# shiivashaakeri/Dynamic-Programming-MultiAgent-Trajectory-Optimiziation

Hardware: AMD Instinct MI355X
Metric: SCvx-iterations/sec, N agents x K=50 nodes (N=1024 per GPU) (higher is better)
Workload: dtype f64

## Files before the change

dynamic-programming-multiagent-trajectory-optimiziation_amd/csrc/qp_factor_phase.hpp:

```cpp
#pragma once
#include "qp_access.hpp"
#include "wave_ops.hpp"

namespace scvx {


struct QPRep {
    int L, R, B, O, G;
    double b1, b2, acc;
};
__device__ __forceinline__ QPRep qp_decode(const int (&d)[4], int one, int lsink, int jnk) {
    QPRep q;
    q.L = d[0] & 0x7FFF;
    q.R = d[1] & 0x7FFF;
    const int bk = d[3] >> 16;
    q.B = bk ? (d[3] & 0x7FFF) : one;
    q.b1 = bk == 1 ? 1.0 : 0.0;
    q.b2 = bk == 2 ? 1.0 : 0.0;
    const int O = d[2];
    const bool on = O >= 0, acc = on && ((O >> 15) & 1);
    q.O = (on && !acc) ? (O & 0x7FFF) : lsink;
    q.acc = acc ? 1.0 : 0.0;
    const int g = on ? (O >> 17) - 1 : -1;
    q.G = (g >= 0 ? g : jnk) * 8;
    return q;
}

template <int KK>
__device__ __forceinline__ double qp_dot(const double* lds, int L, int R) {
    const double* lp = lds + L;
    const double* rp = lds + R;
    double acc0 = 0.0, acc1 = 0.0;
#pragma unroll
    for (int k = 0; k < KK; ++k) {
        if (k & 1) acc1 = fma(lp[k], rp[k], acc1); else acc0 = fma(lp[k], rp[k], acc0);
    }
    return acc0 + acc1;
}

template <int KK, int NREP, int ALO = 0, int AHI = WAVE * NREP>
__device__ __forceinline__ void qp_phase(double* lds, const QPRep (&d)[NREP], double blast, const QPBuf& wb, int fbo,
                                         double (&areg)[NREP]) {
    double val[NREP];
#pragma unroll
    for (int r = 0; r < NREP; ++r)
        val[r] = fma(lds[d[r].B], d[r].b1 + blast * d[r].b2, qp_dot<KK>(lds, d[r].L, d[r].R));
#pragma unroll
    for (int r = 0; r < NREP; ++r) {
        lds[d[r].O] = val[r];
        if (WAVE * r < AHI && WAVE * r + WAVE > ALO) areg[r] = fma(d[r].acc, val[r], areg[r]);
        wb.st(d[r].G, fbo, val[r]);
    }
}

struct QPRepC {
    int LR, BO, GF;
    __device__ __forceinline__ int L() const { return LR & 0xFFFF; }
    __device__ __forceinline__ int R() const { return LR >> 16; }
    __device__ __forceinline__ int B() const { return BO & 0xFFFF; }
    __device__ __forceinline__ int O() const { return BO >> 16; }
    __device__ __forceinline__ int G() const { return GF & 0xFFFF; }
    __device__ __forceinline__ int F() const { return GF >> 16; }
};
__device__ __forceinline__ QPRepC qp_decode_c(const int (&d)[4], int one, int lsink, int jnk) {
    QPRepC q;
    const int L = d[0] & 0x7FFF, R = d[1] & 0x7FFF;
    const int bk = d[3] >> 16;
    const int B = bk ? (d[3] & 0x7FFF) : one;
    const int O = d[2];
    const bool on = O >= 0, acc = on && ((O >> 15) & 1);
    const int Oo = on ? (O & 0x7FFF) : lsink;
    const int g = on ? (O >> 17) - 1 : -1;
    const int G = (g >= 0 ? g : jnk) * 8;
    const int F = bk | (acc ? 4 : 0);
    q.LR = L | (R << 16);
    q.BO = B | (Oo << 16);
    q.GF = G | (F << 16);
    return q;
}
template <int KK, int NREP, int ALO, int AHI>
__device__ __forceinline__ void qp_phase_c(double* lds, const QPRepC* d, double blast, const QPBuf& wb,
                                           int fbo, double (&areg)[NREP]) {
    const QPRepC* q = d;
    double val[NREP];
#pragma unroll
    for (int r = 0; r < NREP; ++r) {
        const int bk = q[r].F() & 3;
        const double bm = (bk == 1 ? 1.0 : 0.0) + blast * (bk == 2 ? 1.0 : 0.0);
        val[r] = fma(lds[q[r].B()], bm, qp_dot<KK>(lds, q[r].L(), q[r].R()));
    }
#pragma unroll
    for (int r = 0; r < NREP; ++r) {
        lds[q[r].O()] = val[r];
        if (WAVE * r < AHI && WAVE * r + WAVE > ALO) areg[r] = fma((q[r].F() & 4) ? 1.0 : 0.0, val[r], areg[r]);
        wb.st(q[r].G(), fbo, val[r]);
    }
}

}
```

dynamic-programming-multiagent-trajectory-optimiziation_amd/csrc/qp_ipm.hpp:

```cpp
#pragma once
#ifndef __HIPCC_RTC__
#include <hip/hip_runtime.h>

#include "common.hpp"
#endif
#include <type_traits>

#include "qp_consts.hpp"
#include "qp_factor_phase.hpp"

namespace scvx {

template <int NX_, int NU_, int NB_, int NO_, int NC_, int VC_ = 0>
struct QPCfg {
    static constexpr QPLay L = qp_layout(NX_, NU_, NB_, NO_, NC_, VC_);
    static_assert(qp_class_error(NX_, NU_, NB_, NO_, NC_, VC_, 2, QP_LDS_DEVICE) == nullptr, "class outside the kernel's limits");
};

struct QPFlagsRT {
    static constexpr bool spec = false;
    static constexpr int has_final = 0, fix_last_input = 0, ineq_last = 0, has_soc = 0, has_coll = 0, n_obs = 0, n_box = 0;
    static constexpr int box_idx(int) { return 0; }
};
template <int FIN, int FIXU, int INEQL, int SOC, int COLL, int NOBS, int NBOX, int B0 = 0, int B1 = 0>
// ... 204 lines not shown
            }
#pragma unroll
            for (int e = 0; e < NX * NU; ++e) pst(C::L.gC + e, Cp[e]);
        }
        const int pd = T.pos_dim;
        double xb[3] = {0, 0, 0};
        for (int i = 0; i < pd; ++i) xb[i] = act ? a.Xref[(agent * K + t) * NX + i] : 0.0;
#pragma unroll
        for (int o = 0; o < NO; ++o) {
            double d[3] = {0, 0, 0}, nr = 0.0, bo = 0.0;
            if (o < nobs) {
                bo = T.obs_radius[o];
#pragma unroll
                for (int i = 0; i < 3; ++i) {
                    d[i] = i < pd ? xb[i] - T.obs_center[o][i] : 0.0;
                    nr += d[i] * d[i];
                }
                nr = sqrt(nr) + 1e-6;
#pragma unroll
                for (int i = 0; i < 3; ++i) {
                    d[i] = d[i] / nr;
                    bo += i < pd ? d[i] * T.obs_center[o][i] : 0.0;
                }
            }
#pragma unroll
            for (int i = 0; i < 3; ++i) cst(C::L.C_SOFT + o * 4 + i, d[i]);
            cst(C::L.C_SOFT + o * 4 + 3, bo);
        }
#pragma unroll
        for (int c = 0; c < NC; ++c) {
            double g[4] = {0, 0, 0, 0};
            if (c < ccount) {
                const double* src = a.coll_rows + ((agent * K + t) * T.j_max + c) * (pd + 1);
                for (int i = 0; i < pd; ++i) g[i] = src[i];
                g[3] = src[pd];
            }
#pragma unroll
            for (int i = 0; i < 4; ++i) cst(C::L.C_SOFT + (NO + c) * 4 + i, g[i]);
        }
#pragma unroll
        for (int j = 0; j < NU; ++j) cst(C::L.C_UB + j, act ? a.Uref[(agent * K + t) * NU + j] : 0.0);
        if (warm) {
            if (lane < 2 * NX) lds[V_YI + lane] = wld(vt, C::L.C_WY * colb);
        } else {
#pragma unroll
            for (int i = 0; i < NX; ++i) {
                cst(C::L.C_Z + i, act ? a.Xref[(agent * K + t) * NX + i] : 0.0);
                cst(C::L.C_Y + i, 0.0);
            }
#pragma unroll
            for (int j = 0; j < NU; ++j) cst(C::L.C_Z + NX + j, act ? a.Uref[(agent * K + t) * NU + j] : 0.0);
#pragma unroll
            for (int g = 0; g < NG; ++g) cst(C::L.C_AV + g, 0.0);
#pragma unroll
            for (int i = 0; i < NV; ++i) { cst(C::L.C_VN + i, 0.0); cst(C::L.C_VE + i, 0.0); }
            if (lane < NX) { lds[V_YI + lane] = 0.0; lds[V_YF + lane] = 0.0; }
        }
        if (lane == 0) lds[V_ONE] = 1.0;
        if (lane < 16) lds[V_ST + lane] = 0.0;
    }
    auto issue_cp = [&](double* Cp) __attribute__((always_inline)) {
#pragma unroll
        for (int e = 0; e < NX * NU; ++e) Cp[e] = wld(vcur - 8, (C::L.C_DT + NX * NX + NX * NU + e) * colb);
    };
    auto take_cp = [&](double* Cp) __attribute__((always_inline)) {
        hold(Cp, NX * NU);
#pragma unroll
        for (int e = 0; e < NX * NU; ++e) Cp[e] = (t > 0) ? Cp[e] : 0.0;
    };
    auto load_cp = [&](double* Cp) __attribute__((always_inline)) {
        issue_cp(Cp);
        take_cp(Cp);
    };
#ifndef QP_RT_STEPS
#define QP_RT_STEPS 15
#endif
    constexpr bool RT_ON = NX <= 8 && NS <= 8 && NV == 0;
    constexpr bool RT_A = RT_ON && (QP_RT_STEPS & 1), RT_B = RT_ON && (QP_RT_STEPS & 2),
                   RT_C = RT_ON && (QP_RT_STEPS & 4), RT_F = RT_ON && (QP_RT_STEPS & 8);

    constexpr int PFN = (PKT + WAVE - 1) / WAVE;
    auto factor = [&](auto phi_issue) __attribute__((always_inline)) -> bool {
        constexpr int E1 = 2 * NX * NX + 2 * NX * NU + 2 * NX, E2 = NX * NX + NU * NX + NU * NU, E4 = 4 * NX * NX;
        constexpr int R1 = (E1 + WAVE - 1) / WAVE, R2 = (E2 + WAVE - 1) / WAVE, R4 = (E4 + WAVE - 1) / WAVE;
        int d1[R1][4], d2[R2][4], d4[R4][4];
        {
            const int sink = C::L.F_SINK;
            const int ln = qp_opaque(lane);
#pragma unroll
            for (int rep = 0; rep < R1; ++rep) {
                int o = ln + rep * WAVE, L = 0, R = 0, O = -1, B = 0;
                if (o < NX * NX) {
                    const int i = o / NX, j = o % NX;
                    L = C::L.F_PP + i * NX; R = C::L.P_A + j * NX; O = C::L.F_T1 + j * NX + i;
                } else if ((o -= NX * NX) < NX * NU) {
                    const int i = o / NU, j = o % NU;
                    L = C::L.F_PP + i * NX; R = C::L.P_BT + j * NX; O = C::L.F_T2 + j * NX + i;
                } else if ((o -= NX * NU) < NX * NX) {
                    const int i = o / NX, j = o % NX;
                    L = C::L.P_A + i * NX; R = C::L.F_PIP + j * NX; O = C::L.F_W1 + o;
                    B = (i == j) ? (V_ONE | (2 << 16)) : 0;
                } else if ((o -= NX * NX) < NU * NX) {
                    const int i = o / NX, j = o % NX;
                    L = C::L.P_BT + i * NX; R = C::L.F_PIP + j * NX;
                    O = (C::L.F_W2 + j * NU + i) | ((C::L.B_W2 + o + 1) << 17);
                    B = (C::L.P_C + i * NX + j) | (1 << 15) | (2 << 16);
                } else if ((o -= NU * NX) < NX) {
                    L = C::L.F_PP + o * NX; R = C::L.P_E; O = sink | ((C::L.B_U + o + 1) << 17);
                } else if ((o -= NX) < NX) {
                    L = C::L.F_PIP + o * NX; R = C::L.P_E; O = (V_XE + o) | (1 << 15);
                }
                d1[rep][0] = L; d1[rep][1] = R; d1[rep][2] = O; d1[rep][3] = B;
            }
#pragma unroll
            for (int rep = 0; rep < R2; ++rep) {
                int o = ln + rep * WAVE, L = 0, R = 0, O = -1, B = 0;
                if (o < NX * NX) {
                    const int i = o / NX, j = o % NX, p = i < j ? i : j, q = i < j ? j : i;
                    L = C::L.P_A + p * NX; R = C::L.F_T1 + q * NX; O = C::L.F_QH + o;
                    B = (C::L.P_Q + p * NX + q) | (1 << 15) | (1 << 16);
                } else if ((o -= NX * NX) < NU * NX) {
                    const int i = o / NX, j = o % NX;
                    L = C::L.P_BT + i * NX; R = C::L.F_T1 + j * NX; O = C::L.F_SH + j * NU + i;
                    B = (C::L.P_S + j * NU + i) | (1 << 15) | (1 << 16);
                } else if ((o -= NU * NX) < NU * NU) {
                    const int i = o / NU, j = o % NU, p = i < j ? i : j, q = i < j ? j : i;
                    L = C::L.P_BT + p * NX; R = C::L.F_T2 + q * NX; O = C::L.F_RH + o;
                    B = (C::L.P_R + p * NU + q) | (1 << 15) | (1 << 16);
                }
                d2[rep][0] = L; d2[rep][1] = R; d2[rep][2] = O; d2[rep][3] = B;
            }
#pragma unroll
            for (int rep = 0; rep < R4; ++rep) {
                int o = ln + rep * WAVE, L = 0, R = 0, O = -1, B = 0;
                if (o < NX * NX) {
                    const int i = o / NX, j = o % NX, p = i < j ? i : j, q = i < j ? j : i;
                    L = C::L.F_SH + p * NU; R = C::L.F_KK + q * NU;
                    O = (C::L.F_PP + o) | ((C::L.B_P + o + 1) << 17); B = (C::L.F_QH + p * NX + q) | (1 << 16);
                } else if ((o -= NX * NX) < NX * NX) {
                    const int i = o / NX, j = o % NX;
                    L = C::L.F_SH + i * NU; R = C::L.F_KK + (NX + j) * NU;
                    O = (C::L.F_PIP + j * NX + i) | ((C::L.B_PI + o + 1) << 17); B = (C::L.F_W1 + o) | (1 << 16);
                } else if ((o -= NX * NX) < NX * NX) {
                    const int i = o / NX, j = o % NX, p = i < j ? i : j, q = i < j ? j : i;
                    L = C::L.F_W2 + p * NU; R = C::L.F_KK + (NX + q) * NU; O = (V_M + o) | (1 << 15);
                } else if ((o -= NX * NX) < NX * NX) {
                    const int i = o / NX, j = o % NX;
                    L = C::L.P_BTR + i * NU; R = C::L.F_KK + j * NU;
                    O = (C::L.NV > 0 ? C::L.F_ACLC + j * NX + i : sink) | ((C::L.B_ACL + o + 1) << 17);
                    B = (C::L.P_A + j * NX + i) | (1 << 15) | (1 << 16);
                }
                d4[rep][0] = L; d4[rep][1] = R; d4[rep][2] = O; d4[rep][3] = B;
            }
        }
        constexpr bool CMP = NX > 8;
        constexpr int RT = R1 + R2 + R4;
        static_assert(!CMP || RT == C::L.NREP, "descriptor table size (QPLay::dtab_doubles, the host's workspace size)");
        const int DTB = FBB + K * C::L.FBS * 8;
        QPRep q1[CMP ? 1 : R1], q2[CMP ? 1 : R2], q4[CMP ? 1 : R4];
        double a1[R1], a2[R2], a4[R4];
        constexpr int R0 = (NX * NX + WAVE - 1) / WAVE;
        double amv[R0];
#pragma unroll
        for (int r = 0; r < R0; ++r) amv[r] = 0.0;
        auto tab_st = [&](int r, const QPRepC& q) __attribute__((always_inline)) {
            qp_u4 w;
            w.x = (unsigned)q.LR; w.y = (unsigned)q.BO; w.z = (unsigned)q.GF; w.w = 0u;
            wb.st4(qp_opaque(lane) * 16, DTB + r * WAVE * 16, w);
        };
        auto tab_ld = [&](int r, int vo) __attribute__((always_inline)) -> QPRepC {
            const qp_u4 w = wb.ld4(vo, DTB + r * WAVE * 16);
            QPRepC q;
            q.LR = (int)w.x; q.BO = (int)w.y; q.GF = (int)w.z;
            return q;
        };
#pragma unroll
        for (int r = 0; r < R1; ++r) {
            if constexpr (CMP) tab_st(r, qp_decode_c(d1[r], V_ONE, C::L.F_SINK, C::L.B_JNK));
            else q1[r] = qp_decode(d1[r], V_ONE, C::L.F_SINK, C::L.B_JNK);
            a1[r] = 0.0;
        }
#pragma unroll
        for (int r = 0; r < R2; ++r) {
            if constexpr (CMP) tab_st(R1 + r, qp_decode_c(d2[r], V_ONE, C::L.F_SINK, C::L.B_JNK));
            else q2[r] = qp_decode(d2[r], V_ONE, C::L.F_SINK, C::L.B_JNK);
            a2[r] = 0.0;
        }
#pragma unroll
        for (int r = 0; r < R4; ++r) {
            if constexpr (CMP) tab_st(R1 + R2 + r, qp_decode_c(d4[r], V_ONE, C::L.F_SINK, C::L.B_JNK));
            else q4[r] = qp_decode(d4[r], V_ONE, C::L.F_SINK, C::L.B_JNK);
            a4[r] = 0.0;
        }
        for (int e = lane; e < NX * NX; e += WAVE) { lds[C::L.F_PP + e] = 0.0; lds[C::L.F_PIP + e] = 0.0; lds[V_M + e] = 0.0; }
        if (lane < NX) lds[V_XE + lane] = 0.0;
        if (lane == 0) { lds[V_FLAG] = 0.0; lds[V_SANY] = 0.0; }
        __syncthreads();
        constexpr int FPD = NX > 8 ? 2 : 3;
        double pf[FPD][PFN];
        int pfo[C::L.DPK ? 1 : PFN];
        if constexpr (!C::L.DPK) {
#pragma unroll
            for (int k = 0; k < PFN; ++k) {
                const int e = qp_opaque(lane) + WAVE * k;
                const int g = e < PKT ? qp_gsrc<C::L>(e) : -1;
                pfo[k] = g >= 0 ? g * 8 : QP_OOB;
            }
        }
        auto pf_load = [&](int ts, double* b) __attribute__((always_inline)) {
            if constexpr (C::L.DPK) {
                const int vo = qp_opaque(lane) * 8;
#pragma unroll
                for (int k = 0; k < PFN; ++k) b[k] = wb.ld(vo, PKB + (ts > 0 ? ts : 0) * C::L.GPK * 8 + k * WAVE * 8);
            } else {
#pragma unroll
                for (int k = 0; k < PFN; ++k) b[k] = wb.ld(pfo[k], PKB + (ts > 0 ? ts : 0) * C::L.GPK * 8);
            }
        };
        auto pf_store = [&](int ts, const double* b) __attribute__((always_inline)) {
            const int sl = NX > 8 ? qp_opaque(lane) : lane;
#pragma unroll
            for (int k = 0; k < PFN; ++k) {
                const int e = sl + WAVE * k;
                lds[e < PKT ? C::L.F_RING + e : C::L.F_SINK] = b[k];
            }
        };
        if constexpr (FPD == 3) {
            pf_load(K - 1, pf[0]);
            pf_load(K - 2, pf[1]);
            pf_load(K - 3, pf[2]);
            pf_store(K - 1, pf[0]);
            pf_load(K - 4, pf[0]);
        } else {
            pf_load(K - 1, pf[0]);
            pf_load(K - 2, pf[1]);
            pf_store(K - 1, pf[0]);
            pf_load(K - 3, pf[0]);
        }
        wsync();
        bool bad = false;
        auto stage = [&](auto lastc, int ts, double* nb, const double* cb) __attribute__((always_inline)) {
            constexpr bool last = decltype(lastc)::value;
            const double blast = last ? 1.0 : 0.0;
            const int fbo = FBB + ts * C::L.FBS * 8;
            const int sl = NX > 8 ? qp_opaque(lane) : lane;
            QPRepC qs[CMP ? RT : 1];
            if constexpr (CMP) {
                const int vo = qp_opaque(lane) * 16;
#pragma unroll
                for (int r = 0; r < RT; ++r) qs[r] = tab_ld(r, vo);
            }
            pf_load(ts - FPD, nb);
            double dfmr = 0.0;
            if constexpr (C::L.STF) dfmr = lds[C::L.F_RING + C::L.P_FD + C::L.NTR + 1 + C::L.NFO];
            if constexpr (C::L.NV > 0) {
                const int c = sl < 4 * NX ? sl : 0, blk = c / NX, cc = c - blk * NX;
                const int base = (blk == 1 ? C::L.F_PIP : C::L.F_PP) + cc * NX;
                const double keep = blk == 2 ? 0.0 : 1.0;
                const double dcc = lds[C::L.F_RING + C::L.P_D + cc];
                const double diag = (blk == 2 ? 1.0 : 0.0) + (blk == 0 ? dcc : 0.0);
                double col[NX];
#pragma unroll
                for (int i = 0; i < NX; ++i) col[i] = fma(keep, lds[base + i], qp_mask(i, cc) * diag);
#pragma unroll
                for (int k = 0; k < NX; ++k) {
                    double pv[NX];
#pragma unroll
                    for (int i = 0; i < NX; ++i) pv[i] = readlane_d(col[i], k);
                    bad |= !(pv[k] > 0.0);
                    const double rk = col[k] / pv[k];
#pragma unroll
                    for (int i = 0; i < NX; ++i) col[i] = (i == k) ? rk : fma(-pv[i], rk, col[i]);
                }
                const bool own = sl >= NX && sl < 4 * NX;
                const int gcol = blk == 1 ? C::L.B_YPI : (blk == 2 ? C::L.B_GI : C::L.B_YP);
#pragma unroll
                for (int i = 0; i < NX; ++i) {
                    const int lo = !own ? C::L.F_SINK + i
                                        : (blk == 1 ? C::L.F_YPI + cc * NX + i
                                                    : (blk == 2 ? C::L.F_Z + i * NX + cc : C::L.F_YP + cc * NX + i));
                    lds[lo] = blk == 2 ? col[i] * dcc : col[i];
                    wb.st((own ? gcol + cc * NX + i : C::L.B_JNK) * 8, fbo, col[i]);
                }
                wsync();
#pragma unroll
                for (int r = 0; r < R0; ++r) {
                    const int o = sl + r * WAVE, oo = o < NX * NX ? o : 0, i = oo / NX, j = oo - i * NX;
                    const double pt = 0.5 * (lds[C::L.F_RING + C::L.P_D + i] * lds[C::L.F_YP + j * NX + i] +
                                             lds[C::L.F_RING + C::L.P_D + j] * lds[C::L.F_YP + i * NX + j]);
                    const double mv = qp_dot<NX>(lds, C::L.F_PIP + i * NX, C::L.F_YPI + j * NX);
                    amv[r] -= o < NX * NX ? mv : 0.0;
                    lds[o < NX * NX ? C::L.F_PP + o : C::L.F_SINK] = pt;
                }
                wsync();
#pragma unroll
                for (int r = 0; r < R0; ++r) {
                    const int o = sl + r * WAVE, oo = o < NX * NX ? o : 0;
                    const double v = lds[C::L.F_RING + C::L.P_D + (oo % NX)] * lds[C::L.F_YPI + oo];
                    lds[o < NX * NX ? C::L.F_PIP + o : C::L.F_SINK] = v;
                }
                wsync();
            }
            pstamp(15);
            if constexpr (CMP) qp_phase_c<NX, R1, E1 - NX, E1>(lds, qs, blast, wb, fbo, a1);
            else qp_phase<NX, R1, E1 - NX, E1>(lds, q1, blast, wb, fbo, a1);
            wsync();
            pstamp(11);
            if constexpr (CMP) qp_phase_c<NX, R2, 0, 0>(lds, qs + R1, blast, wb, fbo, a2);
            else qp_phase<NX, R2, 0, 0>(lds, q2, blast, wb, fbo, a2);
            wsync();
            pstamp(12);
            {
                const bool fx = last && fix_last;
                auto ph3 = [&](auto candc) __attribute__((always_inline)) {
                constexpr bool CAND = decltype(candc)::value;
                constexpr int PM = C::L.PM, PMA = C::L.PMA;
                double Lm[NU * NU], dinv[NU];
#pragma unroll
                for (int e = 0; e < NU * NU; ++e) Lm[e] = lds[C::L.F_RH + e];
                int sfi[PMA];
                double sfd[PMA];
#pragma unroll
                for (int i = 0; i < PMA; ++i) { sfi[i] = -1; sfd[i] = 1.0; }
                bool stg = false;
                if constexpr (C::L.STF && CAND) {
                    constexpr int NTR = C::L.NTR, FS = C::L.F_RING + C::L.P_FD + NTR;
                    {
                    double dnf = 0.0;
#pragma unroll
                    for (int j = 0; j < NU; ++j) dnf = fmax(dnf, fabs(Lm[j * NU + j]));
                    const double thr = QP_STIFF * dnf;
                    {
                        int e = 0;
#pragma unroll
                        for (int i = 0; i < NU; ++i) {
                            Lm[i * NU + i] += lds[FS];
#pragma unroll
                            for (int j = i + 1; j < NU; ++j, ++e) {
                                const double o = lds[FS + 1 + e];
                                Lm[i * NU + j] += o;
                                Lm[j * NU + i] += o;
                            }
                        }
                    }
                    if (__builtin_amdgcn_readfirstlane((int)(dfmr > thr && !fx))) {
                        double Df[NTR];
                        int cnt = 0;
#pragma unroll
                        for (int f = 0; f < NTR; ++f) {
                            Df[f] = lds[C::L.F_RING + C::L.P_FD + f];
                            const bool above = Df[f] > thr;
#pragma unroll
                            for (int i = 0; i < PM; ++i) {
                                sfi[i] = (above && cnt == i) ? f : sfi[i];
                                sfd[i] = (above && cnt == i) ? Df[f] : sfd[i];
                            }
                            cnt += above ? 1 : 0;
                        }
                        bool opp = false;
#pragma unroll
                        for (int i = 0; i < PM; ++i)
#pragma unroll
                            for (int k = i + 1; k < PM; ++k) opp |= sfi[i] >= 0 && sfi[k] >= 0 && (sfi[i] ^ sfi[k]) == NTR - 1;
                        const bool use = cnt <= PM && !opp;
#pragma unroll
                        for (int i = 0; i < PM; ++i) {
                            sfi[i] = use ? sfi[i] : -1;
                            sfd[i] = use ? sfd[i] : 1.0;
                        }
                        if (use) {
#pragma unroll
                            for (int e = 0; e < NU * NU; ++e) Lm[e] = lds[C::L.F_RH + e];
#pragma unroll
                            for (int f = 0; f < NTR; ++f) {
                                bool st = false;
#pragma unroll
                                for (int i = 0; i < PM; ++i) st |= sfi[i] == f;
                                const double d = st ? 0.0 : Df[f];
#pragma unroll
                                for (int i = 0; i < NU; ++i)
#pragma unroll
                                    for (int j = 0; j < NU; ++j) Lm[i * NU + j] += (((f >> i) ^ (f >> j)) & 1) ? -d : d;
                            }
                        }
                        stg = __builtin_amdgcn_readfirstlane((int)use) != 0;
                        if (stg && sl == 0) lds[V_SANY] = 1.0;
                    }
                    }
                }
#ifdef QP_STF_DEBUG
                double Lm0[NU * NU];
#pragma unroll
                for (int e = 0; e < NU * NU; ++e) Lm0[e] = Lm[e];
#endif
                double dmax = 0.0;
#pragma unroll
                for (int j = 0; j < NU; ++j) dmax = fmax(dmax, fabs(Lm[j * NU + j]));
                const double dmin = 1e-13 * dmax + 1e-300;
                bool nan = dmax != dmax;
#pragma unroll
                for (int j = 0; j < NU; ++j) {
                    double d = Lm[j * NU + j];
#pragma unroll
                    for (int k = 0; k < j; ++k) d -= Lm[j * NU + k] * Lm[j * NU + k] * Lm[k * NU + k];
                    nan |= d != d;
                    d = d > dmin ? d : dmin;
                    Lm[j * NU + j] = d;
                    double rq = __builtin_amdgcn_rcp(d);
                    rq = fma(fma(-d, rq, 1.0), rq, rq);
                    dinv[j] = fma(fma(-d, rq, 1.0), rq, rq);
#pragma unroll
                    for (int i = j + 1; i < NU; ++i) {
                        double v = Lm[i * NU + j];
#pragma unroll
                        for (int k = 0; k < j; ++k) v -= Lm[i * NU + k] * Lm[j * NU + k] * Lm[k * NU + k];
                        Lm[i * NU + j] = v * dinv[j];
                    }
                }
                bad |= nan;
                if (fx) {
#pragma unroll
                    for (int e = 0; e < NU * NU; ++e) Lm[e] = (e / NU == e % NU) ? 1.0 : 0.0;
#pragma unroll
                    for (int j = 0; j < NU; ++j) dinv[j] = 1.0;
                }
                auto ldl_solve = [&](double* x) __attribute__((always_inline)) {
#pragma unroll
                    for (int i = 0; i < NU; ++i) {
#pragma unroll
                        for (int k = 0; k < i; ++k) x[i] -= Lm[i * NU + k] * x[k];
                    }
#pragma unroll
                    for (int i = 0; i < NU; ++i) x[i] *= dinv[i];
#pragma unroll
                    for (int i = NU - 1; i >= 0; --i) {
#pragma unroll
                        for (int k = i + 1; k < NU; ++k) x[i] -= Lm[k * NU + i] * x[k];
                    }
                };
                double Wm[NU * PMA], Ci[PMA * PMA];
#pragma unroll
                for (int e = 0; e < NU * PMA; ++e) Wm[e] = 0.0;
#pragma unroll
                for (int e = 0; e < PMA * PMA; ++e) Ci[e] = (e / PMA == e % PMA) ? 1.0 : 0.0;
                if (C::L.STF && CAND && stg) {
#pragma unroll
                    for (int i = 0; i < PM; ++i) {
                        double w[NU];
#pragma unroll
                        for (int j = 0; j < NU; ++j) w[j] = sfi[i] < 0 ? 0.0 : (((sfi[i] >> j) & 1) ? -1.0 : 1.0);
                        ldl_solve(w);
#pragma unroll
                        for (int j = 0; j < NU; ++j) Wm[j * PM + i] = w[j];
                    }
                    double Cm[PMA * PMA];
#pragma unroll
                    for (int i = 0; i < PM; ++i)
#pragma unroll
                        for (int k = 0; k < PM; ++k) {
                            double v = (i == k) ? (sfi[i] < 0 ? 1.0 : 1.0 / sfd[i]) : 0.0;
#pragma unroll
                            for (int j = 0; j < NU; ++j)
                                v += (sfi[i] < 0 ? 0.0 : (((sfi[i] >> j) & 1) ? -1.0 : 1.0)) * Wm[j * PM + k];
                            Cm[i * PM + k] = v;
                        }
#ifdef QP_STF_DEBUG
                    double Cm0[PMA * PMA];
#pragma unroll
                    for (int e = 0; e < PM * PM; ++e) Cm0[e] = Cm[e];
#endif
#pragma unroll
                    for (int e = 0; e < PM * PM; ++e) Ci[e] = (e / PM == e % PM) ? 1.0 : 0.0;
#pragma unroll
                    for (int k = 0; k < PM; ++k) {
                        const double pv = Cm[k * PM + k];
                        bad |= !(pv > 0.0 && __builtin_isfinite(pv));
#ifdef QP_STF_DEBUG
                        if (sl == 0 && !(pv > 0.0 && __builtin_isfinite(pv))) {
                            printf("STF agent %lld stage %d pivot %d = %.6e | C %.6e %.6e %.6e %.6e | sfi %d %d sfd %.3e %.3e | "
                                   "W %.3e %.3e %.3e %.3e %.3e %.3e\n", agent, ts, k, pv, Cm0[0], Cm0[1], Cm0[2], Cm0[3],
                                   sfi[0], sfi[PMA > 1 ? 1 : 0], sfd[0], sfd[PMA > 1 ? 1 : 0], Wm[0], Wm[1], Wm[2],
                                   Wm[3 % (NU * PMA)], Wm[4 % (NU * PMA)], Wm[5 % (NU * PMA)]);
                            printf("STF agent %lld stage %d R0 (folded, before LDL) %.6e %.6e %.6e | %.6e %.6e %.6e | %.6e %.6e %.6e"
                                   " | Rhat %.6e %.6e %.6e %.6e %.6e %.6e %.6e %.6e %.6e | dinv %.6e %.6e %.6e | L %.6e %.6e %.6e\n",
                                   agent, ts, Lm0[0], Lm0[1 % (NU * NU)], Lm0[2 % (NU * NU)], Lm0[3 % (NU * NU)],
                                   Lm0[4 % (NU * NU)], Lm0[5 % (NU * NU)], Lm0[6 % (NU * NU)], Lm0[7 % (NU * NU)],
                                   Lm0[8 % (NU * NU)], lds[C::L.F_RH + 0], lds[C::L.F_RH + 1], lds[C::L.F_RH + 2],
                                   lds[C::L.F_RH + 3], lds[C::L.F_RH + 4 % (NU * NU)], lds[C::L.F_RH + 5 % (NU * NU)],
                                   lds[C::L.F_RH + 6 % (NU * NU)], lds[C::L.F_RH + 7 % (NU * NU)], lds[C::L.F_RH + 8 % (NU * NU)], dinv[0],
                                   dinv[1 % NU], dinv[2 % NU], Lm[3 % (NU * NU)], Lm[6 % (NU * NU)], Lm[7 % (NU * NU)]);
                            double Df8[8];
                            for (int f = 0; f < 8; ++f) Df8[f] = f < C::L.NTR ? lds[C::L.F_RING + C::L.P_FD + f] : 0.0;
                            printf("STF agent %lld stage %d facets D %.3e %.3e %.3e %.3e %.3e %.3e %.3e %.3e\n", agent, ts,
                                   Df8[0], Df8[1], Df8[2], Df8[3], Df8[4], Df8[5], Df8[6], Df8[7]);
                        }
#endif
                        const double rp = 1.0 / pv;
#pragma unroll
                        for (int j = 0; j < PM; ++j) { Cm[k * PM + j] *= rp; Ci[k * PM + j] *= rp; }
#pragma unroll
                        for (int i = 0; i < PM; ++i) {
                            if (i == k) continue;
                            const double f = Cm[i * PM + k];
#pragma unroll
                            for (int j = 0; j < PM; ++j) {
                                Cm[i * PM + j] = fma(-f, Cm[k * PM + j], Cm[i * PM + j]);
                                Ci[i * PM + j] = fma(-f, Ci[k * PM + j], Ci[i * PM + j]);
                            }
                        }
                    }
#pragma unroll
                    for (int e = 0; e < PM * PM; ++e) bad |= !__builtin_isfinite(Ci[e]);
#ifdef QP_STF_DEBUG
                    for (int e = 0; e < PM * PM; ++e)
                        if (sl == 0 && !__builtin_isfinite(Ci[e])) printf("STF agent %lld stage %d Ci[%d] = %.6e\n", agent, ts, e, Ci[e]);
#endif
                }
                {
                    const bool kl = sl < 2 * NX;
                    const int c = kl ? sl : 0;
                    const int off = c < NX ? C::L.F_SH + c * NU : C::L.F_W2 + (c - NX) * NU;
                    double x[NU];
#pragma unroll
                    for (int i = 0; i < NU; ++i) x[i] = lds[off + i];
                    ldl_solve(x);
                    if constexpr (C::L.STF) {
                        double gx[PMA], zc[PMA];
#pragma unroll
                        for (int i = 0; i < PMA; ++i) zc[i] = 0.0;
                        if (CAND && stg) {
#pragma unroll
                        for (int i = 0; i < PM; ++i) {
                            double v = 0.0;
#pragma unroll
                            for (int j = 0; j < NU; ++j)
                                v += (sfi[i] < 0 ? 0.0 : (((sfi[i] >> j) & 1) ? -1.0 : 1.0)) * x[j];
                            gx[i] = v;
                        }
#pragma unroll
                        for (int i = 0; i < PM; ++i) {
                            double v = 0.0;
#pragma unroll
                            for (int k = 0; k < PM; ++k) v = fma(Ci[i * PM + k], gx[k], v);
                            zc[i] = v;
                        }
#pragma unroll
                        for (int j = 0; j < NU; ++j)
#pragma unroll
                            for (int i = 0; i < PM; ++i) x[j] = fma(-Wm[j * PM + i], zc[i], x[j]);
                        }
                        const int gb = c < NX ? C::L.B_GAM + c : C::L.B_GAK + c - NX;
#pragma unroll
                        for (int i = 0; i < PM; ++i) wb.st((kl ? gb + i * NX : C::L.B_JNK) * 8, fbo, fx ? 0.0 : -zc[i]);
                    }
                    const int g = c < NX ? C::L.B_K + c : C::L.B_KAP + c - NX;
#pragma unroll
                    for (int i = 0; i < NU; ++i) {
                        const double v = fx ? 0.0 : -x[i];
                        lds[kl ? C::L.F_KK + c * NU + i : C::L.F_SINK] = v;
                        wb.st((kl ? g + i * NX : C::L.B_JNK) * 8, fbo, v);
                    }
                }
                {
                    double v = 0.0;
#pragma unroll
                    for (int e = 0; e < NU * NU; ++e) {
                        const int ei = e / NU, ej = e % NU;
                        if (ei >= ej) v = (sl == e) ? (ei > ej ? Lm[e] : dinv[ei]) : v;
                    }
                    wb.st((sl < NU * NU ? C::L.B_LD + sl : C::L.B_JNK) * 8, fbo, v);
                }
                if constexpr (C::L.STF) {
                    double v = 0.0;
#pragma unroll
                    for (int e = 0; e < NU * PM; ++e) v = (sl == e) ? Wm[e] : v;
#pragma unroll
                    for (int e = 0; e < PM * PM; ++e) v = (sl == NU * PM + e) ? Ci[e] : v;
#pragma unroll
                    for (int e = 0; e < PM; ++e) v = (sl == NU * PM + PM * PM + e) ? (double)sfi[e] : v;
                    wb.st((sl < C::L.NSMB ? C::L.B_WS + sl : C::L.B_JNK) * 8, fbo, v);
                }
                };
                if constexpr (C::L.STF) {
                    if (__builtin_amdgcn_readfirstlane((int)(dfmr > 0.0))) ph3(std::true_type{});
                    else ph3(std::false_type{});
                } else {
                    ph3(std::false_type{});
                }
            }
            wsync();
            pstamp(13);
            if constexpr (CMP) qp_phase_c<NU, R4, 2 * NX * NX, 3 * NX * NX>(lds, qs + R1 + R2, blast, wb, fbo, a4);
            else qp_phase<NU, R4, 2 * NX * NX, 3 * NX * NX>(lds, q4, blast, wb, fbo, a4);
            if (ts > 0) pf_store(ts - 1, cb);
            wsync();
            pstamp(14);
            if constexpr (C::L.NV > 0) {
#pragma unroll
                for (int r = 0; r < R0; ++r) {
                    const int o = sl + r * WAVE, oo = o < NX * NX ? o : 0, i = oo / NX, j = oo - i * NX;
                    const double v = qp_dot<NX>(lds, C::L.F_Z + i * NX, C::L.F_ACLC + j * NX);
                    wb.st((o < NX * NX ? C::L.B_ACL2 + o : C::L.B_JNK) * 8, fbo, v);
                }
                wsync();
            }
        };
        int ts = K - 1;
        if constexpr (FPD == 3) {
            stage(std::true_type{}, ts, pf[0], pf[1]);
            --ts;
            while (ts >= 0) {
                stage(std::false_type{}, ts, pf[1], pf[2]);
                if (--ts < 0) break;
                stage(std::false_type{}, ts, pf[2], pf[0]);
                if (--ts < 0) break;
                stage(std::false_type{}, ts, pf[0], pf[1]);
                --ts;
            }
        } else {
            stage(std::true_type{}, ts, pf[0], pf[1]);
            --ts;
            while (ts >= 0) {
                stage(std::false_type{}, ts, pf[1], pf[0]);
                if (--ts < 0) break;
                stage(std::false_type{}, ts, pf[0], pf[1]);
                --ts;
            }
        }
        if (bad) lds[V_FLAG] = 1.0;
        if constexpr (CMP) {
            const int vo = qp_opaque(lane) * 16;
#pragma unroll
            for (int r = 0; r < R1; ++r) {
                if (WAVE * r < E1 && WAVE * r + WAVE > E1 - NX) {
                    const QPRepC q = tab_ld(r, vo);
                    if (q.F() & 4) lds[q.O()] = a1[r];
                }
            }
#pragma unroll
            for (int r = 0; r < R4; ++r) {
                if (WAVE * r < 3 * NX * NX && WAVE * r + WAVE > 2 * NX * NX) {
                    const QPRepC q = tab_ld(R1 + R2 + r, vo);
                    if (q.F() & 4) lds[q.O()] = a4[r];
                }
            }
        } else {
#pragma unroll
            for (int r = 0; r < R1; ++r)
                if (d1[r][2] >= 0 && ((d1[r][2] >> 15) & 1)) lds[d1[r][2] & 0x7FFF] = a1[r];
#pragma unroll
            for (int r = 0; r < R4; ++r)
                if (d4[r][2] >= 0 && ((d4[r][2] >> 15) & 1)) lds[d4[r][2] & 0x7FFF] = a4[r];
        }
        wsync();
        if constexpr (C::L.NV > 0) {
#pragma unroll
            for (int r = 0; r < R0; ++r) {
                const int o = lane + r * WAVE;
                if (o < NX * NX) lds[V_M + o] += amv[r];
            }
            wsync();
        }
        for (int e = lane; e < NX * NX; e += WAVE) lds[V_PI0 + e] = lds[C::L.F_PIP + (e % NX) * NX + e / NX];
        if constexpr (NX > 8) {
            if (fin) {
                const int j = lane < NX ? lane : 0;
                double col[NX];
#pragma unroll
                for (int i = 0; i < NX; ++i) col[i] = lds[V_M + i * NX + j];
#pragma unroll
                for (int k = 0; k < NX; ++k) {
                    double ck[NX];
#pragma unroll
                    for (int i = 0; i < NX; ++i) ck[i] = readlane_d(col[i], k);
                    int p = k;
                    double best = fabs(ck[k]);
#pragma unroll
                    for (int i = k + 1; i < NX; ++i) {
                        const double v = fabs(ck[i]);
                        if (v > best) { best = v; p = i; }
                    }
                    if (lane == 0) lds[V_PIV + k] = (double)p;
#pragma unroll
                    for (int i = k + 1; i < NX; ++i) {
                        const double m = qp_mask(i, p);
                        const double dlt = m * (col[i] - col[k]);
                        col[k] += dlt;
                        col[i] -= dlt;
                    }
#pragma unroll
                    for (int i = 0; i < NX; ++i) ck[i] = readlane_d(col[i], k);
                    const double d = ck[k];
                    if (lane == 0 && (d == 0.0 || d != d)) lds[V_FLAG] = 2.0;
                    const double inv = d != 0.0 ? 1.0 / d : 0.0;
#pragma unroll
                    for (int i = k + 1; i < NX; ++i) {
                        const double f = ck[i] * inv;
                        col[i] = (j == k) ? f : ((j > k) ? col[i] - f * col[k] : col[i]);
                    }
                }
                if (lane < NX)
#pragma unroll
                    for (int i = 0; i < NX; ++i) lds[V_M + i * NX + j] = col[i];
            }
        } else {
        if (fin && lane == 0) {
            double Mr[NX * NX];
#pragma unroll
            for (int e = 0; e < NX * NX; ++e) Mr[e] = lds[V_M + e];
#pragma unroll
            for (int k = 0; k < NX; ++k) {
                int p = k;
                double best = fabs(Mr[k * NX + k]);
#pragma unroll
                for (int i = k + 1; i < NX; ++i) {
                    const double v = fabs(Mr[i * NX + k]);
                    if (v > best) { best = v; p = i; }
                }
                lds[V_PIV + k] = (double)p;
#pragma unroll
                for (int i = k + 1; i < NX; ++i) {
                    const double m = qp_mask(i, p);
#pragma unroll
                    for (int j = 0; j < NX; ++j) {
                        const double dlt = m * (Mr[i * NX + j] - Mr[k * NX + j]);
                        Mr[k * NX + j] += dlt;
                        Mr[i * NX + j] -= dlt;
                    }
                }
                const double d = Mr[k * NX + k];
                if (d == 0.0 || d != d) lds[V_FLAG] = 2.0;
                const double inv = d != 0.0 ? 1.0 / d : 0.0;
#pragma unroll
                for (int i = k + 1; i < NX; ++i) {
                    const double f = Mr[i * NX + k] * inv;
                    Mr[i * NX + k] = f;
#pragma unroll
                    for (int j = k + 1; j < NX; ++j) Mr[i * NX + j] -= f * Mr[k * NX + j];
                }
            }
#pragma unroll
            for (int e = 0; e < NX * NX; ++e) lds[V_M + e] = Mr[e];
        }
        }
        wsync();
        if constexpr (C::L.CHK) {
            const ChunkC cc = chunk_coords();
            const int ch = cc.ch, ce = cc.ce, cs0 = cc.cs0, cs1 = cc.cs1;
            const bool cact = cc.act;
            double ar[QP_CLM][NX], ph[NX];
#pragma unroll
            for (int j = 0; j < QP_CLM; ++j) {
                const int tj = cs0 + j;
                const int vo = (cact && j < CL && tj < cs1) ? (C::L.B_CH + ce * NX) * 8 + tj * C::L.FBS * 8 : QP_OOB;
#pragma unroll
                for (int k = 0; k < NX; ++k) {
                    if constexpr (NX % 2 == 0) { if (!(k & 1)) wld2(&ar[j][k], vo, FBB, k * 8); }
                    else ar[j][k] = wld(vo, FBB, k * 8);
                }
            }
            phi_issue();
#pragma unroll
            for (int c = 0; c < NX; ++c) ph[c] = (c == ce) ? 1.0 : 0.0;
#pragma unroll
            for (int j = 0; j < QP_CLM; ++j) {
                if (j < CL) {
                    double nw[NX];
#pragma unroll
                    for (int c = 0; c < NX; ++c) nw[c] = 0.0;
#pragma unroll
                    for (int k = 0; k < NX; ++k)
#pragma unroll
                        for (int c = 0; c < NX; ++c) nw[c] = fma(ar[j][k], oct_bcast_d(ph[c], k), nw[c]);
                    const bool ok = cs0 + j < cs1;
#pragma unroll
                    for (int c = 0; c < NX; ++c) ph[c] = ok ? nw[c] : ph[c];
                }
            }
#pragma unroll
            for (int c = 0; c < NX; ++c) lds[cact ? V_PHI + ch * NX * NX + ce * NX + c : C::L.F_SINK] = ph[c];
            wsync();
        }
        return lds[V_FLAG] == 0.0;
    };

    auto solve = [&](const double* q, const double* r, const double* dv, double* dzo, double* dyo, double* dno,
                     const double* rhs_s, double* fnu) __attribute__((always_inline)) {
        constexpr int PM = C::L.PM, PMA = C::L.PMA;
        double g0[PMA];
#pragma unroll
        for (int i = 0; i < PMA; ++i) { g0[i] = 0.0; fnu[i] = 0.0; }
        fresh();
        if (act) {
            double g[NX], u[NX];
            ldb(u, C::L.B_U, NX);
            if constexpr (NV > 0) {
                double Y[NX * NX];
                ldb(Y, C::L.B_YP, NX * NX);
                hold(u, NX);
                hold(Y, NX * NX);
#pragma unroll
                for (int j = 0; j < NX; ++j)
#pragma unroll
                    for (int i = 0; i < NX; ++i) u[j] = fma(-Y[j * NX + i], dv[i], u[j]);
            }
            double Kt[NU * NX], Ac[NX * NX];
            ldb(Kt, C::L.B_K, NU * NX);
            ldb(Ac, C::L.B_ACL, NX * NX);
            hold(Kt, NU * NX);
            hold(u, NX);
            hold(Ac, NX * NX);
#pragma unroll
            for (int i = 0; i < NX; ++i) g[i] = q[i];
            if constexpr (C::L.STF) {
                if (stf_any()) {
                    double Gm[PMA * NX];
                    ldb(Gm, C::L.B_GAM, PM * NX);
                    hold(Gm, PM * NX);
#pragma unroll
                    for (int i = 0; i < PM; ++i)
#pragma unroll
                        for (int j = 0; j < NX; ++j) g[j] = fma(-Gm[i * NX + j], rhs_s[i], g[j]);
                }
            }
#pragma unroll
            for (int i = 0; i < NU; ++i)
#pragma unroll
                for (int j = 0; j < NX; ++j) g[j] = fma(Kt[i * NX + j], r[i], g[j]);
            if (t < K - 1) {
#pragma unroll
                for (int i = 0; i < NX; ++i)
#pragma unroll
                    for (int j = 0; j < NX; ++j) g[j] = fma(Ac[i * NX + j], u[i], g[j]);
            }
#pragma unroll
            for (int i = 0; i < NX; ++i) lds[V_G + t * NX + i] = g[i];
        }
        wsync();
        stamp(4);
        constexpr int HC = RT_C ? 1 : 0;
        double hU[HC * NX + 1 - HC], hBt[HC * NX * NU + 1 - HC], hLd[HC * NU * NU + 1 - HC], hW2[HC * NU * NX + 1 - HC];
        double hKap[HC * NU * NX + 1 - HC], hPi[HC * NX * NX + 1 - HC], hEv[HC * NX + 1 - HC];
        double hKt[HC * NU * NX + 1 - HC], hP[HC * NX * NX + 1 - HC], hCp[HC * NX * NU + 1 - HC];
        auto issue_bpost = [&](double* uu, double* Bt, double* Ld, double* W2) __attribute__((always_inline)) {
            ldb(uu, C::L.B_U, NX);
            ldn(Bt, C::L.C_BT, NX * NU);
            ldb(Ld, C::L.B_LD, NU * NU);
            ldb(W2, C::L.B_W2, NU * NX);
        };
        auto issue_fpre = [&](double* kap, double* Pi, double* Bt, double* ev) __attribute__((always_inline)) {
            ldb(kap, C::L.B_KAP, NU * NX);
            ldb(Pi, C::L.B_PI, NX * NX);
            if (Bt) ldn(Bt, C::L.C_BT, NX * NU);
#pragma unroll
            for (int i = 0; i < NX; ++i) ev[i] = pld(C::L.gE + i);
        };
        auto issue_fpost = [&](double* Kt, double* P, double* Cp) __attribute__((always_inline)) {
            ldb(Kt, C::L.B_K, NU * NX);
            ldb(P, C::L.B_P, NX * NX);
            issue_cp(Cp);
        };
        if constexpr (C::L.CHK) {
            const ChunkC cc = chunk_coords();
            const int ce = cc.ce, cs0 = cc.cs0, cs1 = cc.cs1;
            const bool cact = cc.act;
            double ac[QP_CLM][NX], gc[QP_CLM];
#pragma unroll
            for (int j = 0; j < QP_CLM; ++j) {
                const int tj = cs1 - 1 - j;
                const bool ok = cact && j < CL && tj >= cs0;
                const int vo = ok ? (C::L.B_CH + ce) * 8 + tj * C::L.FBS * 8 : QP_OOB;
#pragma unroll
                for (int k = 0; k < NX; ++k) ac[j][k] = wld(vo, FBB, k * NX * 8);
                gc[j] = lds[V_G + (ok ? tj : 0) * NX + (ce < NX ? ce : 0)];
            }
            if constexpr (RT_C) issue_bpost(hU, hBt, hLd, hW2);
            auto chainT = [&](double q, const double* a, double g) __attribute__((always_inline)) -> double {
                double v0 = g, v1 = 0.0;
#pragma unroll
                for (int k = 0; k < NX; ++k) {
                    const double qk = oct_bcast_d(q, k);
                    if (k & 1) v1 = fma(a[k], qk, v1); else v0 = fma(a[k], qk, v0);
                }
                return v0 + v1;
            };
            const double gK = lds[V_G + (K - 1) * NX + (ce < NX ? ce : 0)];
            if (lane < NX) lds[V_CH + (K - 1) * NX + lane] = gK;
            double q = (cs1 == KS) ? gK : 0.0;
#pragma unroll
            for (int j = 0; j < QP_CLM; ++j) {
                if (j < CL) {
                    const double qn = chainT(q, ac[j], gc[j]);
                    q = (cs1 - 1 - j >= cs0) ? qn : q;
                }
            }
            lds[cact ? V_CH + cs0 * NX + ce : C::L.F_SINK] = q;
// ... 1718 lines not shown
```

Measured before the change: 186.5.

## Prefetch LDS operands of factor phases ahead of barriers into registers

Splits each factorization phase into an issue step that loads all LDS operands into registers and a finish step that does the dot products. Operands that are already final (the left operand and bias of phase 2 and of phase 4) are loaded early, before the preceding barrier or during the Cholesky step. This hides LDS latency behind earlier work. Empty asm constraints pin the loaded values so the compiler cannot sink the loads back. A per-class mask selects the path, and some shapes are excluded. The cost is higher register pressure and possibly lower occupancy.

```diff
diff --git a/dynamic-programming-multiagent-trajectory-optimiziation_amd/csrc/qp_factor_phase.hpp b/dynamic-programming-multiagent-trajectory-optimiziation_amd/csrc/qp_factor_phase.hpp
--- a/dynamic-programming-multiagent-trajectory-optimiziation_amd/csrc/qp_factor_phase.hpp
+++ b/dynamic-programming-multiagent-trajectory-optimiziation_amd/csrc/qp_factor_phase.hpp
@@ -38,18 +38,77 @@
     return acc0 + acc1;
 }
 
-template <int KK, int NREP, int ALO = 0, int AHI = WAVE * NREP>
-__device__ __forceinline__ void qp_phase(double* lds, const QPRep (&d)[NREP], double blast, const QPBuf& wb, int fbo,
-                                         double (&areg)[NREP]) {
+#ifndef QP_FS_STEPS
+#define QP_FS_STEPS 3
+#endif
+constexpr int QP_FS_A = 1, QP_FS_C = 2;
+constexpr int qp_fs_mask(int nx, int nu, int nb, int no, int nc) {
+    int m = nx > 8 ? 0 : QP_FS_STEPS;
+    if (nx == 3 && nu == 2 && nc == 32) m = 0;
+    if (nx == 6 && nb == 2 && no == 0 && nc == 16) m &= QP_FS_A;
+    return m;
+}
+
+__device__ __forceinline__ void qp_pin(double& v) { asm volatile("" : "+v"(v)); }
+
+template <int KK, int NREP>
+struct QPOps {
+    double l[NREP][KK], r[NREP][KK], b[NREP];
+};
+template <int SEL, int KK, int NREP>
+__device__ __forceinline__ void qp_phase_issue(const double* lds, const QPRep (&d)[NREP], QPOps<KK, NREP>& o) {
+#pragma unroll
+    for (int r = 0; r < NREP; ++r) {
+#pragma unroll
+        for (int k = 0; k < KK; ++k) {
+            if (SEL & 1) o.l[r][k] = lds[d[r].L + k];
+            if (SEL & 2) o.r[r][k] = lds[d[r].R + k];
+        }
+        if (SEL & 1) o.b[r] = lds[d[r].B];
+    }
+}
+template <int KK, int NREP, int ALO, int AHI>
+__device__ __forceinline__ void qp_phase_finish(double* lds, const QPRep (&d)[NREP], double blast, const QPBuf& wb, int fbo,
+                                                double (&areg)[NREP], QPOps<KK, NREP>& o) {
     double val[NREP];
 #pragma unroll
-    for (int r = 0; r < NREP; ++r)
-        val[r] = fma(lds[d[r].B], d[r].b1 + blast * d[r].b2, qp_dot<KK>(lds, d[r].L, d[r].R));
+    for (int r = 0; r < NREP; ++r) {
+        double acc0 = 0.0, acc1 = 0.0;
+#pragma unroll
+        for (int k = 0; k < KK; ++k) {
+            qp_pin(o.l[r][k]);
+            qp_pin(o.r[r][k]);
+            if (k & 1) acc1 = fma(o.l[r][k], o.r[r][k], acc1); else acc0 = fma(o.l[r][k], o.r[r][k], acc0);
+        }
+        qp_pin(o.b[r]);
+        val[r] = fma(o.b[r], d[r].b1 + blast * d[r].b2, acc0 + acc1);
+    }
 #pragma unroll
     for (int r = 0; r < NREP; ++r) {
         lds[d[r].O] = val[r];
         if (WAVE * r < AHI && WAVE * r + WAVE > ALO) areg[r] = fma(d[r].acc, val[r], areg[r]);
         wb.st(d[r].G, fbo, val[r]);
+    }
+}
+
+template <int FSM, int KK, int NREP, int ALO = 0, int AHI = WAVE * NREP>
+__device__ __forceinline__ void qp_phase(double* lds, const QPRep (&d)[NREP], double blast, const QPBuf& wb, int fbo,
+                                         double (&areg)[NREP]) {
+    if constexpr ((FSM & QP_FS_A) != 0) {
+        QPOps<KK, NREP> o;
+        qp_phase_issue<3>(lds, d, o);
+        qp_phase_finish<KK, NREP, ALO, AHI>(lds, d, blast, wb, fbo, areg, o);
+    } else {
+        double val[NREP];
+#pragma unroll
+        for (int r = 0; r < NREP; ++r)
+            val[r] = fma(lds[d[r].B], d[r].b1 + blast * d[r].b2, qp_dot<KK>(lds, d[r].L, d[r].R));
+#pragma unroll
+        for (int r = 0; r < NREP; ++r) {
+            lds[d[r].O] = val[r];
+            if (WAVE * r < AHI && WAVE * r + WAVE > ALO) areg[r] = fma(d[r].acc, val[r], areg[r]);
+            wb.st(d[r].G, fbo, val[r]);
+        }
     }
 }
 
diff --git a/dynamic-programming-multiagent-trajectory-optimiziation_amd/csrc/qp_ipm.hpp b/dynamic-programming-multiagent-trajectory-optimiziation_amd/csrc/qp_ipm.hpp
--- a/dynamic-programming-multiagent-trajectory-optimiziation_amd/csrc/qp_ipm.hpp
+++ b/dynamic-programming-multiagent-trajectory-optimiziation_amd/csrc/qp_ipm.hpp
@@ -530,12 +530,30 @@
                 wsync();
             }
             pstamp(15);
-            if constexpr (CMP) qp_phase_c<NX, R1, E1 - NX, E1>(lds, qs, blast, wb, fbo, a1);
-            else qp_phase<NX, R1, E1 - NX, E1>(lds, q1, blast, wb, fbo, a1);
+            constexpr int FSM = qp_fs_mask(NX, NU, C::L.NB, C::L.NO, C::L.NC);
+            constexpr bool FS_E = (FSM & QP_FS_C) != 0;
+            QPOps<NX, CMP ? 1 : R2> o2;
+            QPOps<NU, CMP ? 1 : R4> o4;
+            if constexpr (CMP) {
+                qp_phase_c<NX, R1, E1 - NX, E1>(lds, qs, blast, wb, fbo, a1);
+            } else if constexpr (FS_E) {
+                QPOps<NX, R1> o1;
+                qp_phase_issue<3>(lds, q1, o1);
+                qp_phase_issue<1>(lds, q2, o2);
+                qp_phase_finish<NX, R1, E1 - NX, E1>(lds, q1, blast, wb, fbo, a1, o1);
+            } else {
+                qp_phase<FSM, NX, R1, E1 - NX, E1>(lds, q1, blast, wb, fbo, a1);
+            }
             wsync();
             pstamp(11);
-            if constexpr (CMP) qp_phase_c<NX, R2, 0, 0>(lds, qs + R1, blast, wb, fbo, a2);
-            else qp_phase<NX, R2, 0, 0>(lds, q2, blast, wb, fbo, a2);
+            if constexpr (CMP) {
+                qp_phase_c<NX, R2, 0, 0>(lds, qs + R1, blast, wb, fbo, a2);
+            } else if constexpr (FS_E) {
+                qp_phase_issue<2>(lds, q2, o2);
+                qp_phase_finish<NX, R2, 0, 0>(lds, q2, blast, wb, fbo, a2, o2);
+            } else {
+                qp_phase<FSM, NX, R2, 0, 0>(lds, q2, blast, wb, fbo, a2);
+            }
             wsync();
             pstamp(12);
             {
@@ -546,6 +564,7 @@
                 double Lm[NU * NU], dinv[NU];
 #pragma unroll
                 for (int e = 0; e < NU * NU; ++e) Lm[e] = lds[C::L.F_RH + e];
+                if constexpr (FS_E) qp_phase_issue<1>(lds, q4, o4);
                 int sfi[PMA];
                 double sfd[PMA];
 #pragma unroll
@@ -818,8 +837,14 @@
             }
             wsync();
             pstamp(13);
-            if constexpr (CMP) qp_phase_c<NU, R4, 2 * NX * NX, 3 * NX * NX>(lds, qs + R1 + R2, blast, wb, fbo, a4);
-            else qp_phase<NU, R4, 2 * NX * NX, 3 * NX * NX>(lds, q4, blast, wb, fbo, a4);
+            if constexpr (CMP) {
+                qp_phase_c<NU, R4, 2 * NX * NX, 3 * NX * NX>(lds, qs + R1 + R2, blast, wb, fbo, a4);
+            } else if constexpr (FS_E) {
+                qp_phase_issue<2>(lds, q4, o4);
+                qp_phase_finish<NU, R4, 2 * NX * NX, 3 * NX * NX>(lds, q4, blast, wb, fbo, a4, o4);
+            } else {
+                qp_phase<FSM, NU, R4, 2 * NX * NX, 3 * NX * NX>(lds, q4, blast, wb, fbo, a4);
+            }
             if (ts > 0) pf_store(ts - 1, cb);
             wsync();
             pstamp(14);
```

Result: faster. 192.8, median of 6 (+3.4%).
